# baker-laboratory/NA-MPNN

Hardware: AMD Instinct MI355X
Metric: residues/sec (enc+dec fwd), N~1000 K=48 h=128; seq-recovery vs CPU ref (higher is better)
Workload: dtype f32; 1 GPU; cfg2: B=1 x N=1000 residues per rank, K=48, H=128, 3 enc + 3 dec layers, per-edge GEMMs fp32, seeded random-init weights, independent complexes per rank; precision=fp32, global_batch=1, seq_len=1000, parallelism=replicas x1

## Files before the change

### na_mpnn_amd/csrc/namp.hip

```cpp
#include "../../include/namp.h"
#include "namp_kernels.h"
#include <atomic>
#include "namp_bf16s32.h"
#include "namp_bf16p.h"
#include "namp_node_w.h"
#include "namp_order.h"

#include <cstdarg>
#include <cstdlib>
#include <initializer_list>
#include <cstdio>
#include <mutex>
#include <vector>

namespace {

thread_local char g_err[512] = "";

int fail(int code, const char* fmt, ...) {
  va_list ap;
  va_start(ap, fmt);
  vsnprintf(g_err, sizeof(g_err), fmt, ap);
  va_end(ap);
  return code;
// ... 296 lines not shown
    if (e.npw <= 8 && 2 * e.npw <= e.nwaves) return launch_edge<MODE, 8, PREC_X3, PRE>(a, s);
    return launch_edge<MODE, 16, PREC_X3, PRE>(a, s);
  }
  if (e.npw <= 4) return launch_edge<MODE, 4, PREC_F32, PRE>(a, s);
  if (e.npw <= 8 && 2 * e.npw <= e.nwaves) return launch_edge<MODE, 8, PREC_F32, PRE>(a, s);
  return launch_edge<MODE, 16, PREC_F32, PRE>(a, s);
}

void fill_tail(NodeTail& t, const float* ln1_g, const float* ln1_b, const float* Win_img, const float* b_in,
               const float* Wout_img, const float* b_out, const float* ln2_g, const float* ln2_b, const float* hV,
               const int32_t* mask, float* hV_out, const NampProj* proj, int nproj, const int32_t* S) {
  t.hV = hV; t.mask = mask; t.ln1_g = ln1_g; t.ln1_b = ln1_b; t.Win_img = Win_img; t.b_in = b_in;
  t.Wout_img = Wout_img; t.b_out = b_out; t.ln2_g = ln2_g; t.ln2_b = ln2_b; t.hV_out = hV_out; t.S = S;
  t.head_w = nullptr; t.head_b = nullptr; t.log_probs = nullptr; t.logits = nullptr; t.vocab = 0;
  t.m3_img = nullptr; t.m3_b = nullptr;
  t.nproj = nproj;
  for (int i = 0; i < 8; ++i) {
    if (i < nproj) { t.p[i].img = proj[i].img; t.p[i].bias = proj[i].bias; t.p[i].tok = proj[i].tok; t.p[i].out = proj[i].out; }
    else { t.p[i].img = nullptr; t.p[i].bias = nullptr; t.p[i].tok = nullptr; t.p[i].out = nullptr; }
  }
}

int check_proj(const char* fn, const NampProj* proj, int nproj, const int32_t* S) {
  if (nproj < 0 || nproj > 8 || (nproj > 0 && !proj)) return fail(NAMP_EINVAL, "%s: nproj=%d must be in [0,8]", fn, nproj);
  for (int i = 0; i < nproj; ++i) {
    if (!proj[i].img || !proj[i].out) return fail(NAMP_EINVAL, "%s: proj[%d] has a null image / output", fn, i);
    if (!aligned16(proj[i].img) || !aligned16(proj[i].out) || !aligned16(proj[i].bias) || !aligned16(proj[i].tok))
      return fail(NAMP_EINVAL, "%s: proj[%d] pointers must be 16-byte aligned", fn, i);
    if (proj[i].tok && !S) return fail(NAMP_EINVAL, "%s: proj[%d].tok given but S is null", fn, i);
  }
  return NAMP_OK;
}

struct Out16Req { __bf16* p[8]; int n; bool honoured; };
thread_local Out16Req* g_out16 = nullptr;
thread_local bool g_residue_x1 = false;

int launch_node_linear(const float* X, const int32_t* S, int G_out, int G_src, int N,
                       const NampProj* proj, int nproj, const NampProj* pre, hipStream_t s, bool x3 = false, unsigned* zero = nullptr) {
  NodeLinearArgs a;
  a.X = X; a.S = S; a.G_out = G_out; a.G_src = G_src; a.N = N; a.nproj = nproj; a.zero = zero;
  a.pre.img = pre ? pre->img : nullptr; a.pre.bias = pre ? pre->bias : nullptr;
  a.pre.tok = nullptr; a.pre.out = pre ? pre->out : nullptr;
  for (int i = 0; i < 8; ++i) {
    const NampProj& p = proj[i < nproj ? i : 0];
    a.p[i].img = p.img; a.p[i].bias = p.bias; a.p[i].tok = p.tok; a.p[i].out = p.out;
    a.out16[i] = (g_out16 && i < nproj && i < g_out16->n) ? g_out16->p[i] : nullptr;
    if (a.out16[i]) a.p[i].out = nullptr;
  }
  if (g_out16) g_out16->honoured = true;
  const int units = ((G_out + 15) / 16) * nproj;
  if (x3 && G_out >= 4096 && (g_bf16p.load(std::memory_order_relaxed) & 8) && ensure_attributes() == NAMP_OK) {
    if (g_residue_x1) hipLaunchKernelGGL(node_linear_w_kernel<2>, dim3((G_out + NODEW_ROWS - 1) / NODEW_ROWS), dim3(NODEW_THREADS), NODEW_LDS, s, a);
    else hipLaunchKernelGGL(node_linear_w_kernel<1>, dim3((G_out + NODEW_ROWS - 1) / NODEW_ROWS), dim3(NODEW_THREADS), NODEW_LDS, s, a);
    return NAMP_OK;
  }
  if (x3 && g_residue_x1) hipLaunchKernelGGL(node_linear_kernel<2>, dim3((units + 3) / 4), dim3(256), 0, s, a);
  else if (x3) hipLaunchKernelGGL(node_linear_kernel<1>, dim3((units + 3) / 4), dim3(256), 0, s, a);
  else hipLaunchKernelGGL(node_linear_kernel<0>, dim3((units + 3) / 4), dim3(256), 0, s, a);
  return NAMP_OK;
}

int launch_node_update(const float* ln1_g, const float* ln1_b, const float* Win_img, const float* b_in,
                       const float* Wout_img, const float* b_out, const float* ln2_g, const float* ln2_b,
                       const float* hV, const float* partial, const float* m3_img, const float* m3_b, const int32_t* mask,
                       float* hV_out, const NampProj* proj, int nproj, const int32_t* S, int G, int TPN, hipStream_t s,
// ... 1439 lines not shown
    };
    int cur_ = 0;
    for (int l = 0; l < 3; ++l) {
      const NampEncLayerW* L = &w->enc[l];
      const bool last = (l == 2);
      StageArgs& st = PA_.st[l];
      common(st);
      const int tm = (l & 1) ? 4 : 0, tn = (l & 1) ? 0 : 4, te = (l & 1) ? 6 : 2, tp = (l & 1) ? 2 : 6;
      st.Pa = P[tm]; st.Pj0 = P[tm + 1]; st.Pj1 = nullptr;
      st.W1_img = pick_img(prec, L->W1b_img, nullptr, L->W1b_ximg); st.W2_img = pick_img(prec, L->W2_img, nullptr, L->W2_ximg);
      st.W3_img = pick_img(prec, L->W3_img, nullptr, L->W3_ximg); st.b2 = L->b2; st.b3 = L->b3;
      REQUIRE_PTR(st.W1_img); REQUIRE_PTR(st.W2_img); REQUIRE_PTR(st.W3_img); REQUIRE_PTR(st.b2); REQUIRE_PTR(st.b3);
      if (l == 0) {
        if (E) { st.eW1_img = pick_img(prec, w->We_img, nullptr, w->We_ximg); st.eb2 = w->We_b; REQUIRE_PTR(st.eW1_img); REQUIRE_PTR(st.eb2); }
      } else {
        const NampEncLayerW* Lp = &w->enc[l - 1];
        st.ePa = P[tp]; st.ePj = P[tp + 1];
        st.eW1_img = pick_img(prec, Lp->W11b_img, nullptr, Lp->W11b_ximg); st.eW2_img = pick_img(prec, Lp->W12_img, nullptr, Lp->W12_ximg);
        st.eW3_img = pick_img(prec, Lp->W13_img, nullptr, Lp->W13_ximg); st.eb2 = Lp->b12; st.eb3 = Lp->b13;
        st.ln_g = Lp->ln3_g; st.ln_b = Lp->ln3_b;
        REQUIRE_PTR(st.eW1_img); REQUIRE_PTR(st.eW2_img); REQUIRE_PTR(st.eW3_img); REQUIRE_PTR(st.ln_g); REQUIRE_PTR(st.ln_b);
      }
      st.hE_out = nullptr;
      NampProj pe[8];
      int np = 0;
      pe[np++] = {L->W11a_img, L->b11, nullptr, P[te]};
      pe[np++] = {L->W11c_img, nullptr, nullptr, P[te + 1]};
      if (!last) {
        const NampEncLayerW* Ln = &w->enc[l + 1];
        pe[np++] = {Ln->W1a_img, Ln->b1, nullptr, P[tn]};
        pe[np++] = {Ln->W1c_img, nullptr, nullptr, P[tn + 1]};
      } else {
        const NampDecLayerW* D0 = &w->dec[0];
        for (int d = 0; d < 3; ++d) pe[np++] = {w->dec[d].W1v_img, nullptr, nullptr, Pfw[d]};
        pe[np++] = {D0->W1a_img, D0->b1, nullptr, PA[0]};
        pe[np++] = {D0->W1v_img, nullptr, D0->tok, PB[0]};
      }
      if ((rc = check_proj(__func__, pe, np, S))) return rc;
      fill_tail(st.tail, L->ln1_g, L->ln1_b, L->Win_img, L->b_in, L->Wout_img, L->b_out, L->ln2_g, L->ln2_b, hv[cur_], mask,
                last ? h_V : hv[cur_ ^ 1], pe, np, S);
      st.tail.m3_img = L->W3_img; st.tail.m3_b = L->b3;
      cur_ ^= 1;
    }
    const float* hin_ = h_V;
    for (int l = 0; l < 3; ++l) {
      const NampDecLayerW* D = &w->dec[l];
      StageArgs& st = PA_.st[3 + l];
      common(st);
      st.Pa = PA[l & 1]; st.Pj0 = PB[l & 1]; st.Pj1 = Pfw[l];
      st.W1_img = pick_img(prec, D->W1e_img, nullptr, D->W1e_ximg); st.W2_img = pick_img(prec, D->W2_img, nullptr, D->W2_ximg);
      st.W3_img = pick_img(prec, D->W3_img, nullptr, D->W3_ximg); st.b2 = D->b2; st.b3 = D->b3;
      REQUIRE_PTR(st.W1_img); REQUIRE_PTR(st.W2_img); REQUIRE_PTR(st.W3_img); REQUIRE_PTR(st.b2); REQUIRE_PTR(st.b3);
      if (l == 0) {
        const NampEncLayerW* Lp = &w->enc[2];
        st.ePa = P[2]; st.ePj = P[3];
        st.eW1_img = pick_img(prec, Lp->W11b_img, nullptr, Lp->W11b_ximg); st.eW2_img = pick_img(prec, Lp->W12_img, nullptr, Lp->W12_ximg);
        st.eW3_img = pick_img(prec, Lp->W13_img, nullptr, Lp->W13_ximg); st.eb2 = Lp->b12; st.eb3 = Lp->b13;
        st.ln_g = Lp->ln3_g; st.ln_b = Lp->ln3_b;
        REQUIRE_PTR(st.eW1_img); REQUIRE_PTR(st.eW2_img); REQUIRE_PTR(st.eW3_img); REQUIRE_PTR(st.ln_g); REQUIRE_PTR(st.ln_b);
        st.hE_out = h_E;
      }
      NampProj pn[2] = {{}, {}};
      int np = 0;
      if (l < 2) {
        const NampDecLayerW* Dn = &w->dec[l + 1];
        pn[np++] = {Dn->W1a_img, Dn->b1, nullptr, PA[(l + 1) & 1]};
        pn[np++] = {Dn->W1v_img, nullptr, Dn->tok, PB[(l + 1) & 1]};
      }
      if ((rc = check_proj(__func__, pn, np, S))) return rc;
      fill_tail(st.tail, D->ln1_g, D->ln1_b, D->Win_img, D->b_in, D->Wout_img, D->b_out, D->ln2_g, D->ln2_b, hin_, mask, dhv[l & 1],
                pn, np, S);
      st.tail.m3_img = D->W3_img; st.tail.m3_b = D->b3;
      if (l == 2) { st.tail.head_w = w->Wout_w; st.tail.head_b = w->Wout_b; st.tail.log_probs = log_probs; st.tail.logits = logits; st.tail.vocab = w->vocab; }
      hin_ = dhv[l & 1];
    }
    {
      ProfScope prof_(NAMP_KIND_ENCDEC_PERSISTENT, s);
      if ((rc = namp_internal_launch_persistent(&PA_, prec == PREC_X3 ? 1 : 0, eg.grid, eg.nwaves * 64, s)))
        return fail(NAMP_ELAUNCH, "namp_encdec_fwd: persistent launch setup failed (%d)", rc);
    }
    CHECK_LAUNCH();
    persist_mark(s, pdev);
    return NAMP_OK;
  }
  int cur = 0;
  for (int l = 0; l < w->n_enc; ++l) {
    const NampEncLayerW* L = &w->enc[l];
    const bool last = (l + 1 == w->n_enc);
    float* out = last ? h_V : hv[cur ^ 1];
    const int tm = (l & 1) ? 4 : 0, tn = (l & 1) ? 0 : 4, te = (l & 1) ? 6 : 2, tp = (l & 1) ? 2 : 6;
    NampProj pe[8];
    int np = 0;
    pe[np++] = {L->W11a_img, L->b11, nullptr, P[te]};
    pe[np++] = {L->W11c_img, nullptr, nullptr, P[te + 1]};
    if (!last) {
      const NampEncLayerW* Ln = &w->enc[l + 1];
      pe[np++] = {Ln->W1a_img, Ln->b1, nullptr, P[tn]};
      pe[np++] = {Ln->W1c_img, nullptr, nullptr, P[tn + 1]};
    } else {
      const NampDecLayerW* D0 = &w->dec[0];
      for (int d = 0; d < w->n_dec; ++d) pe[np++] = {w->dec[d].W1v_img, nullptr, nullptr, Pfw[d]};
      pe[np++] = {D0->W1a_img, D0->b1, nullptr, PA[0]};
      pe[np++] = {D0->W1v_img, nullptr, D0->tok, PB[0]};
    }
    if ((rc = check_proj(__func__, pe, np, S))) return rc;
    EdgeArgs a = {};
    a.hE = h_E; a.E_idx = E_idx; a.mask = mask; a.Pa = P[tm]; a.Pj0 = P[tm + 1];
    a.W1_img = pick_img(prec, L->W1b_img, nullptr, L->W1b_ximg); a.W2_img = pick_img(prec, L->W2_img, nullptr, L->W2_ximg);
    a.W3_img = pick_img(prec, L->W3_img, nullptr, L->W3_ximg); a.b2 = L->b2; a.b3 = L->b3;
    REQUIRE_PTR(a.W1_img); REQUIRE_PTR(a.W2_img); REQUIRE_PTR(a.W3_img);
    a.G = a.G_enc = G; a.N = N; a.K = K;
    fill_tail(a.tail, L->ln1_g, L->ln1_b, L->Win_img, L->b_in, L->Wout_img, L->b_out, L->ln2_g, L->ln2_b, hv[cur], mask, out,
              pe, np, S);
    a.tail.m3_img = L->W3_img; a.tail.m3_b = L->b3;
    if (l == 0 && E) {
      a.hE = E; a.hE_out = h_E; a.eW1_img = pick_img(prec, w->We_img, nullptr, w->We_ximg); a.eb2 = w->We_b;
      REQUIRE_PTR(a.eW1_img);
      ProfScope prof_(NAMP_KIND_ENC_MESSAGE, s);
      rc = launch_edge_tail_fused<MODE_ENC_MSG, PRE_EMBED>(a, prec, s);
    } else if (l == 0) {
      ProfScope prof_(NAMP_KIND_ENC_MESSAGE, s);
      rc = launch_edge_tail<MODE_ENC_MSG>(a, prec, s);
    } else {
      const NampEncLayerW* Lp = &w->enc[l - 1];
      a.hE_out = h_E; a.ePa = P[tp]; a.ePj = P[tp + 1];
      a.eW1_img = pick_img(prec, Lp->W11b_img, nullptr, Lp->W11b_ximg); a.eW2_img = pick_img(prec, Lp->W12_img, nullptr, Lp->W12_ximg);
      a.eW3_img = pick_img(prec, Lp->W13_img, nullptr, Lp->W13_ximg); a.eb2 = Lp->b12; a.eb3 = Lp->b13;
      REQUIRE_PTR(a.eW1_img); REQUIRE_PTR(a.eW2_img); REQUIRE_PTR(a.eW3_img);
      a.ln_g = Lp->ln3_g; a.ln_b = Lp->ln3_b;
      ProfScope prof_(NAMP_KIND_ENC_EDGE_MESSAGE, s);
      rc = launch_edge_tail_fused<MODE_ENC_MSG>(a, prec, s);
    }
    if (rc) return rc;
    CHECK_LAUNCH();
    cur ^= 1;
  }
  const int te_last = ((w->n_enc - 1) & 1) ? 6 : 2;
  const float* hin = h_V;
  for (int l = 0; l < w->n_dec; ++l) {
    const NampDecLayerW* D = &w->dec[l];
    const bool last = (l + 1 == w->n_dec);
    float* out = dhv[l & 1];
    NampProj pn[2] = {{}, {}};
    int np = 0;
    if (!last) {
      const NampDecLayerW* Dn = &w->dec[l + 1];
      pn[0] = {Dn->W1a_img, Dn->b1, nullptr, PA[(l + 1) & 1]};
// ... 126 lines not shown
```

### na_mpnn_amd/csrc/namp_kernels.h

```cpp
#pragma once
#include "namp_device.h"
#ifndef NAMP_MAX_LAYERS
#define NAMP_MAX_LAYERS 8
#endif

static __global__ void pack_image_kernel(const float* __restrict__ W, int ld, int col0, int OUT, int IN,
                                  float* __restrict__ img) {
  const int total = OUT * IN;
  for (int e = blockIdx.x * blockDim.x + threadIdx.x; e < total; e += gridDim.x * blockDim.x) {
    const int r = e & 3, lane = (e >> 2) & 63, t = e >> 8;
    const int ntn = OUT >> 4;
    const int tn = t % ntn, tk = t / ntn;
    const int n = 16 * tn + (lane & 15), k = 16 * tk + 4 * (lane >> 4) + r;
    img[e] = W[(size_t)n * ld + col0 + k];
  }
}

static __global__ void pack_image_bf16_kernel(const float* __restrict__ W, int ld, int col0, __bf16* __restrict__ img) {
  const int e = blockIdx.x * blockDim.x + threadIdx.x;
  if (e >= 128 * 128) return;
  const int j = e & 7, lane = (e >> 3) & 63, tn = (e >> 9) & 7, s = e >> 12;
  const int n = 16 * tn + (lane & 15), k = 32 * s + 16 * (j >> 2) + 4 * (lane >> 4) + (j & 3);
  img[e] = (__bf16)W[(size_t)n * ld + col0 + k];
}
// ... 88 lines not shown
          const long b = row / NK;
          const long j = b * N + idx[row];
          v[u] = *(const f4*)(nodes + j * C2 + 4 * (s - s1));
        }
      }
    }
#pragma unroll
    for (int u = 0; u < UNROLL; ++u) {
      if (e0 + u * stride < total) __builtin_nontemporal_store(v[u], (f4*)(out + 4 * (base + e0 + u * stride)));
    }
  }
}

static __global__ void gather_cat_scalar_kernel(const float* __restrict__ nodes, const float* __restrict__ nbrs,
                                         const int32_t* __restrict__ idx, float* __restrict__ out,
                                         long rows, int NK, int N, int C1, int C2) {
  const int ct = C1 + C2;
  const long total = rows * ct;
  for (long e = (long)blockIdx.x * blockDim.x + threadIdx.x; e < total; e += (long)gridDim.x * blockDim.x) {
    const long row = e / ct;
    const int c = (int)(e - row * ct);
    out[e] = (c < C1) ? nbrs[row * C1 + c] : nodes[((row / NK) * N + idx[row]) * C2 + (c - C1)];
  }
}

struct ProjDesc {
  const float* img;
  const float* bias;
  const float* tok;
  float* out;
};

struct NodeTail {
  const float* hV;
  const int32_t* mask;
  const float* ln1_g; const float* ln1_b;
  const float* Win_img;
  const float* b_in;
  const float* Wout_img;
  const float* b_out;
  const float* ln2_g; const float* ln2_b;
  float* hV_out;
  const int32_t* S;
  const float* m3_img;
  const float* m3_b;
  const float* head_w;
  const float* head_b;
  float* log_probs;
  float* logits;
  int vocab;
  int nproj;
  ProjDesc p[8];
};

__device__ __forceinline__ void tail_head_row(const NodeTail& a, const float* ybase, const int sc, const int orow,
                                              const int lane) {
  float z = -INFINITY;
  if (lane < a.vocab) {
    const float* w = a.head_w + (long)lane * NAMP_H;
    float s0 = 0.f, s1 = 0.f, s2 = 0.f, s3 = 0.f;
#pragma unroll 8
    for (int c = 0; c < NAMP_H; c += 4) {
      const f4 wv = *(const f4*)(w + c);
      s0 = fmaf(wv.x, ybase[(c + 0) * sc], s0); s1 = fmaf(wv.y, ybase[(c + 1) * sc], s1);
      s2 = fmaf(wv.z, ybase[(c + 2) * sc], s2); s3 = fmaf(wv.w, ybase[(c + 3) * sc], s3);
    }
    z = (s0 + s1) + (s2 + s3) + a.head_b[lane];
  }
  float mx = z;
#pragma unroll
  for (int o = 1; o < 64; o <<= 1) mx = fmaxf(mx, __shfl_xor(mx, o));
  float e = (lane < a.vocab) ? expf(z - mx) : 0.f;
#pragma unroll
  for (int o = 1; o < 64; o <<= 1) e += __shfl_xor(e, o);
  if (lane < a.vocab) {
    a.log_probs[(long)orow * a.vocab + lane] = (z - mx) - logf(e);
    if (a.logits) a.logits[(long)orow * a.vocab + lane] = z;
  }
}

#define FFN_LD 132
#define NODE_TAIL_LDS ((16 + 16 + 8 * 16) * FFN_LD * 4)
// ... 438 lines not shown
      if (orw >= 0) tail_head_row(a, yT + n, R, orw, lane);
    }
  }
  f4 xr[NB][8];
  tail4_x<NB>(xr, yB, lane);
  int orw[NB];
#pragma unroll
  for (int nb = 0; nb < NB; ++nb) orw[nb] = orow(4 * nb + j);
  auto proj_out = [&](const f4 (&o)[NB], const float* bias, const float* tok, float* out, const int tn) {
    if (!st_lane) return;
    const int c = 16 * tn + 4 * cb;
    const f4 b = bias ? *(const f4*)(bias + c) : (f4){0.f, 0.f, 0.f, 0.f};
#pragma unroll
    for (int nb = 0; nb < NB; ++nb) {
      if (orw[nb] < 0) continue;
      f4 r = o[nb] + b;
      if (tok) r += *(const f4*)(tok + (long)a.S[orw[nb]] * NAMP_H + c);
      float* dst = out + (long)orw[nb] * NAMP_H + c;
      if (SC1) { st_out<true>(dst, r.x); st_out<true>(dst + 1, r.y); st_out<true>(dst + 2, r.z); st_out<true>(dst + 3, r.w); }
      else *(f4*)dst = r;
    }
  };
  if constexpr (PF) {
    tail_units<true>(wave, 8 * (a.nproj < 2 ? a.nproj : 2), nwaves, lane,
                     [&](const int v, const int tk) { return (const f4*)((v >> 3) ? a.p[1].img : a.p[0].img) + (tk * 8 + (v & 7)) * 64; },
                     [&](const int v, const f4 (&wf)[8]) {
                       const bool second = (v >> 3) != 0;
                       f4 o[NB];
                       tail4_unit<NB>(o, wf, xr);
                       proj_out(o, second ? a.p[1].bias : a.p[0].bias, second ? a.p[1].tok : a.p[0].tok, second ? a.p[1].out : a.p[0].out, v & 7);
                     });
    return;
  }
#pragma unroll
  for (int pi = 0; pi < 8; ++pi) {
    if (pi >= a.nproj) break;
    const ProjDesc pd = a.p[pi];
    bool first = AHEAD && pi < TAIL4_AHEAD;
#pragma unroll 1
    for (int tn = ((wave - pi * 8) % nwaves + nwaves) % nwaves; tn < 8; tn += nwaves) {
      f4 o[NB];
      if (first) {
        tail4_unit<NB>(o, wa[pi < TAIL4_AHEAD ? pi : 0], xr);
      } else {
        f4 wf[8];
#pragma unroll
        for (int tk = 0; tk < 8; ++tk) wf[tk] = ((const f4*)pd.img)[(tk * 8 + tn) * 64 + lane];
        tail4_unit<NB>(o, wf, xr);
      }
      first = false;
      proj_out(o, pd.bias, pd.tok, pd.out, tn);
    }
  }
}

template <int R, typename RowFn, bool SC1 = false, bool M3 = true, bool PF = false, bool AH = false>
__device__ __forceinline__ void node_tail_rows(const NodeTail& a, f4 (&x)[8], const float wsum_m, const RowFn orow, float* lds,
                                               const int tid, const int wave, const int nwaves, const int lane) {
#ifndef NAMP_TAIL_VALU
  node_tail_mfma4<R, RowFn, SC1, M3, PF, AH>(a, x, wsum_m, orow, lds, tid, wave, nwaves, lane);
  return;
#endif
  float* xT = lds;
  float* hT = xT + 128 * R;
  float* oP = hT + 512 * R;
  float* yT = oP + 4 * 128 * R;
  float* red = yT + 128 * R;
  const int m = lane & 15, g = lane >> 4;

  if (M3 && a.m3_img) {
    if (wave == 0 && m < R) {
#pragma unroll
      for (int t = 0; t < 8; ++t) {
        xT[(16 * t + 4 * g + 0) * R + m] = x[t].x; xT[(16 * t + 4 * g + 1) * R + m] = x[t].y;
        xT[(16 * t + 4 * g + 2) * R + m] = x[t].z; xT[(16 * t + 4 * g + 3) * R + m] = x[t].w;
      }
      if (g == 0) red[m] = wsum_m;
    }
    __syncthreads();
#pragma unroll 1
    for (int tn = wave; tn < 8; tn += nwaves) {
      f4 wf[8];
#pragma unroll
      for (int tk = 0; tk < 8; ++tk) wf[tk] = ((const f4*)a.m3_img)[(tk * 8 + tn) * 64 + lane];
// ... 264 lines not shown
    }
  }
  if (a.nproj > 0) {
#pragma unroll
    for (int s = 0; s < 4; ++s) split_x3(x[2 * s], x[2 * s + 1], xh[s], xm[s]);
#pragma unroll
    for (int pi = 0; pi < 2; ++pi) {
      if (pi >= a.nproj) break;
      const bf8* wp = (const bf8*)(pi ? p1_p : p0_p) + lane;
      const int tn = wave;
      bf8 f[8];
#pragma unroll
      for (int s = 0; s < 4; ++s) { f[2 * s] = wp[(s * 8 + tn) * 64]; f[2 * s + 1] = wp[NAMP_BIMG_BYTES / 16 + (s * 8 + tn) * 64]; }
      f4 acc = a.p[pi].bias ? *(const f4*)(a.p[pi].bias + 16 * tn + 4 * g) : (f4){0.f, 0.f, 0.f, 0.f};
#pragma unroll
      for (int s = 0; s < 4; ++s) acc = mfma_x3(f[2 * s], f[2 * s + 1], xh[s], xm[s], acc);
      if (orw >= 0) {
        if (a.p[pi].tok) acc += *(const f4*)(a.p[pi].tok + (long)a.S[orw] * NAMP_H + 16 * tn + 4 * g);
        st_f4<SC1>(a.p[pi].out + (long)orw * NAMP_H + 16 * tn + 4 * g, acc);
      }
    }
  }
}

enum { MODE_ENC_MSG = 0, MODE_DEC_MSG = 1, MODE_ENC_EDGE = 2, MODE_EMBED = 3 };

typedef __bf16 bf4 __attribute__((ext_vector_type(4)));
__device__ __forceinline__ int frag_off(const int t, const int g) { return 16 * t + 8 * (g & 1) + 4 * (g >> 1); }
__device__ __forceinline__ void st_frag4(__bf16* row, const int t, const int g, const f4 v) {
  *(bf4*)(row + frag_off(t, g)) = (bf4){(__bf16)v.x, (__bf16)v.y, (__bf16)v.z, (__bf16)v.w};
}

struct EdgeArgs {
  const float* hE;
  float* hE_out;
  const int32_t* E_idx;
  const int32_t* mask;
  const int32_t* mask_attend;
  const int32_t* rank;
  const float* Pa;
  const float* Pj0;
  const float* Pj1;
  const float* W1_img;
  const float* W2_img;
  const float* W3_img;
  const float* b1;
  const float* b2;
  const float* b3;
  const float* ln_g;
  const float* ln_b;
  const float* ePa; const float* ePj;
  const float* eW1_img; const float* eW2_img; const float* eW3_img;
  const float* eb2; const float* eb3;
  uint32_t drop_thresh, drop_seed; float drop_scale;
  const __bf16* hE16; __bf16* hE16_out;
  const __bf16* Pa16; const __bf16* Pj016; const __bf16* Pj116;
  float* partial;
  NodeTail tail;
  int G;
  int G_enc;
  int N, K, TPN;
};

#define EDGE_TAIL_LDS (2 * NAMP_IMG_BYTES + 12 * NAMP_H * 4 + 64 + 2048)

enum { PRE_NONE = 0, PRE_EMBED = 1, PRE_EDGE = 3 };
enum { PREC_F32 = 0, PREC_BF16 = 1, PREC_X3 = 2 };
template <int MODE, int TAIL, int PREC, int PRE, int PERSIST, class Args>
__device__ __forceinline__ void edge_stage(const Args& a, f4 (&x)[8], char* smem) {
  f4 l2pf0 = (f4){0.f, 0.f, 0.f, 0.f}, l2pf1 = l2pf0;
  constexpr bool BF16 = (PREC == PREC_BF16);
  constexpr bool X3 = (PREC == PREC_X3);
  static_assert(PRE == PRE_NONE || (!BF16 && TAIL != 0 && (MODE == MODE_ENC_MSG || MODE == MODE_DEC_MSG)), "PRE: fp32-class message + tail only");
  constexpr bool FUSE = (PRE == PRE_EDGE);
  constexpr bool MSG = (MODE == MODE_ENC_MSG || MODE == MODE_DEC_MSG);
  constexpr bool M3_LDS = MSG && !BF16 && (TAIL == 4 || TAIL == 8);
  char* buf0 = smem;
  char* buf1 = smem + NAMP_IMG_BYTES;
  const int tid = threadIdx.x;
  const int lane = tid & 63;
  const int wave = __builtin_amdgcn_readfirstlane(tid >> 6);
  const int nwaves = blockDim.x >> 6;

  const int m = lane & 15, g = lane >> 4;
  const int npw = nwaves / a.TPN;
  const int node_l = wave / a.TPN, kt = wave - node_l * a.TPN;
  const int bid = xcd_block_index(blockIdx.x, gridDim.x);
  int node = bid * npw + node_l;
  const bool wave_active = (node_l < npw) && (node < a.G);
  if (!wave_active) node = 0;
  const int b_dec = node / a.N;
  const int i_loc = node - b_dec * a.N;
  const int node_enc = (MODE == MODE_DEC_MSG) ? ((b_dec % (a.G_enc / a.N)) * a.N + i_loc) : node;
  const int k = 16 * kt + m;
  const bool valid = wave_active && (k < a.K);
  const long erow = (long)node_enc * a.K + (valid ? k : 0);

  f4 acc[8];
  f4 ybuf[8];
  f4 (&y)[8] = PERSIST ? ybuf : x;
  f4 pjv[8];
  float w_row = 0.f;
  if (PERSIST != 2) {
    const float* src = a.hE + erow * NAMP_H + 4 * g;
#pragma unroll
    for (int t = 0; t < 8; ++t) x[t] = *(const f4*)(src + 16 * t);
  }
  if (MODE == MODE_EMBED) {
    if (a.ln_g) layernorm_row_T(x, a.ln_g, a.ln_b, g);
// ... 33 lines not shown

  const f4* w0 = (const f4*)buf0 + lane;
  const f4* w1 = (const f4*)buf1 + lane;

  if (BF16) {
    const bf8* bw = (const bf8*)smem + lane;
    dma_to_lds(smem, a.W1_img, 32, wave, nwaves, lane);
    if (MODE != MODE_EMBED) dma_to_lds(smem + NAMP_BIMG_BYTES, a.W2_img, 32, wave, nwaves, lane);
    if (MODE == MODE_ENC_EDGE) dma_to_lds(smem + 2 * NAMP_BIMG_BYTES, a.W3_img, 32, wave, nwaves, lane);
    wait_dma_and_sync();
    chain_gemm_bf16<false, false>(acc, x, bw);
    if (MODE != MODE_EMBED) {
#pragma unroll
      for (int t = 0; t < 8; ++t) acc[t] += pjv[t];
      if (MSG) {
#pragma unroll
        for (int t = 0; t < 8; ++t) { const float b = a.b2[16 * t + m]; y[t] = (f4){b, b, b, b}; }
        chain_gemm_bf16<true, true>(y, acc, bw + (NAMP_BIMG_BYTES / 16));
      } else {
#pragma unroll
        for (int t = 0; t < 8; ++t) y[t] = *(const f4*)(a.b2 + 16 * t + 4 * g);
        chain_gemm_bf16<false, true>(y, acc, bw + (NAMP_BIMG_BYTES / 16));
      }
    }
  } else {
  float* cstf = (float*)(smem + 2 * NAMP_IMG_BYTES + 12 * NAMP_H * 4 + 64);
  if (FUSE) {
    dma_to_lds(buf1, a.eW1_img, 64, wave, nwaves, lane);
    dma_to_lds(buf0, a.eW2_img, 64, wave, nwaves, lane);
    for (int i = tid; i < 512; i += (int)blockDim.x) {
      const float* srcv = i < 128 ? a.eb2 : i < 256 ? a.eb3 : i < 384 ? a.ln_g : a.ln_b;
      cstf[i] = srcv[i & 127];
    }
    wait_dma_and_sync();
    gemm128<X3, false, false>(acc, x, w1);
#pragma unroll
    for (int t = 0; t < 8; ++t) acc[t] += pjv[t];
    __syncthreads();
    dma_to_lds(buf1, a.eW3_img, 64, wave, nwaves, lane);
#pragma unroll
    for (int t = 0; t < 8; ++t) pjv[t] = *(const f4*)(cstf + 16 * t + 4 * g);
    gemm128<X3, false, true>(pjv, acc, w0);
    wait_dma_and_sync();
    dma_to_lds(buf0, a.W1_img, 64, wave, nwaves, lane);
#pragma unroll
    for (int t = 0; t < 8; ++t) acc[t] = *(const f4*)(cstf + 128 + 16 * t + 4 * g);
    gemm128<X3, false, true>(acc, pjv, w1);
#pragma unroll
    for (int t = 0; t < 8; ++t) x[t] += acc[t];
    layernorm_row_T(x, cstf + 256, cstf + 384, g);
    if (valid && (PERSIST == 0 || a.hE_out != nullptr)) {
      float* dst = a.hE_out + erow * NAMP_H + 4 * g;
#pragma unroll
      for (int t = 0; t < 8; ++t) *(f4*)(dst + 16 * t) = x[t];
    }
  }
  if (PRE != PRE_NONE) {
    if (PRE == PRE_EMBED) {
      dma_to_lds(buf1, a.eW1_img, 64, wave, nwaves, lane);
      dma_to_lds(buf0, a.W1_img, 64, wave, nwaves, lane);
#pragma unroll
      for (int t = 0; t < 8; ++t) acc[t] = *(const f4*)(a.eb2 + 16 * t + 4 * g);
      wait_dma_and_sync();
      gemm128<X3, false, false>(acc, x, w1);
#pragma unroll
      for (int t = 0; t < 8; ++t) x[t] = acc[t];
      if (valid && (PERSIST == 0 || a.hE_out != nullptr)) {
        float* dst = a.hE_out + erow * NAMP_H + 4 * g;
#pragma unroll
        for (int t = 0; t < 8; ++t) *(f4*)(dst + 16 * t) = x[t];
      }
    }
    {
      const int j_loc = a.E_idx[erow];
      const float* pj;
      if (MODE == MODE_DEC_MSG) {
        const int j_dec = b_dec * a.N + j_loc;
        const bool bw = a.rank[j_dec] < a.rank[node];
        pj = bw ? (a.Pj0 + (long)j_dec * NAMP_H) : (a.Pj1 + (long)(node_enc - i_loc + j_loc) * NAMP_H);
        w_row = valid ? (1.0f / 30.0f) : 0.f;
      } else {
        const int j = node - i_loc + j_loc;
        pj = a.Pj0 + (long)j * NAMP_H;
        int ma;
        if (a.mask_attend) ma = a.mask_attend[erow];
        else ma = a.mask ? (a.mask[node] * a.mask[j]) : 1;
        w_row = valid ? ((float)ma * (1.0f / 30.0f)) : 0.f;
      }
      const float* pa = a.Pa + (long)node * NAMP_H + 4 * g;
      pj += 4 * g;
#pragma unroll
      for (int t = 0; t < 8; ++t) { acc[t] = *(const f4*)(pa + 16 * t); pjv[t] = *(const f4*)(pj + 16 * t); }
    }
    if (PRE == PRE_EMBED) __syncthreads();
    else wait_dma_and_sync();
    dma_to_lds(buf1, a.W2_img, 64, wave, nwaves, lane);
  } else {
  dma_to_lds(buf0, a.W1_img, 64, wave, nwaves, lane);
  if (MODE != MODE_EMBED) dma_to_lds(buf1, a.W2_img, 64, wave, nwaves, lane);
  wait_dma_and_sync();
  }
  gemm128<X3, false, false>(acc, x, w0);

  if (MODE != MODE_EMBED) {
#pragma unroll
  for (int t = 0; t < 8; ++t) acc[t] += pjv[t];
  if (MSG) {
    if (PRE != PRE_NONE) wait_dma_and_sync();
    else if (M3_LDS) __syncthreads();
    if (M3_LDS) dma_to_lds(buf0, a.W3_img, 64, wave, nwaves, lane);
    if (TAIL == 4 || TAIL == 8) {
      const int slice = (blockIdx.x >> 3) & 31;
      const f4* p0; const f4* p1;
      if (wave < 8) {
        p0 = (const f4*)a.tail.Win_img + (slice * 8 + wave) * 64; p1 = (const f4*)a.tail.Wout_img + (slice * 8 + wave) * 64;
      } else {
        const int q = wave - 8;
        const float* img = q == 0 ? a.tail.p[0].img : q == 1 ? a.tail.p[1].img : q == 2 ? a.tail.p[2].img : a.tail.p[3].img;
        if (q >= a.tail.nproj) img = a.tail.Win_img;
        p0 = (const f4*)img + (slice * 2) * 64; p1 = p0 + 64;
      }
      l2pf0 = p0[lane]; l2pf1 = p1[lane];
    }
#pragma unroll
    for (int t = 0; t < 8; ++t) { const float b = a.b2[16 * t + m]; y[t] = (f4){b, b, b, b}; }
    gemm128<X3, true, true>(y, acc, w1);
  } else {
  if (PRE != PRE_NONE) wait_dma_and_sync();
  else __syncthreads();
  dma_to_lds(buf0, a.W3_img, 64, wave, nwaves, lane);

#pragma unroll
// ... 132 lines not shown
  unsigned spins = 0;
  while (__hip_atomic_load(word, __ATOMIC_RELAXED, __HIP_MEMORY_SCOPE_AGENT) < target) {
    __builtin_amdgcn_s_sleep(2);
    if (++spins > NAMP_SPIN_LIMIT) {
      __hip_atomic_store(tmo, code, __ATOMIC_RELAXED, __HIP_MEMORY_SCOPE_AGENT);
      return false;
    }
  }
  return true;
}

__device__ __forceinline__ void grid_barrier(unsigned* sync, const unsigned epoch, const int tid) {
  asm volatile("s_waitcnt vmcnt(0)" ::: "memory");
  __syncthreads();
  if (tid == 0) {
    gu32* sy = (gu32*)sync;
    const int grp = blockIdx.x % NAMP_SYNC_GROUPS;
    const unsigned ngroups = gridDim.x < NAMP_SYNC_GROUPS ? gridDim.x : NAMP_SYNC_GROUPS;
    const unsigned in_group = (gridDim.x - grp + NAMP_SYNC_GROUPS - 1) / NAMP_SYNC_GROUPS;
    const unsigned old = __hip_atomic_fetch_add(sy + grp, 1u, __ATOMIC_RELAXED, __HIP_MEMORY_SCOPE_AGENT);
    if (old + 1 == in_group * epoch) {
      __hip_atomic_fetch_add(sy + NAMP_SYNC_TOP, 1u, __ATOMIC_RELAXED, __HIP_MEMORY_SCOPE_AGENT);
      spin_until_ge(sy + NAMP_SYNC_TOP, ngroups * epoch, sy + NAMP_SYNC_TIMEOUT, 0x10000000u | epoch);
      __hip_atomic_store(sy + NAMP_SYNC_GEN + grp, epoch, __ATOMIC_RELAXED, __HIP_MEMORY_SCOPE_AGENT);
    } else {
      spin_until_ge(sy + NAMP_SYNC_GEN + grp, epoch, sy + NAMP_SYNC_TIMEOUT, 0x20000000u | epoch);
    }
    __builtin_amdgcn_fence(__ATOMIC_ACQUIRE, "agent");
  }
  __syncthreads();
}

struct StageArgs {
  const float* hE; float* hE_out; const int32_t* E_idx; const int32_t* mask; const int32_t* rank;
  const float* Pa; const float* Pj0; const float* Pj1;
  const float* W1_img; const float* W2_img; const float* W3_img; const float* b2; const float* b3;
  const float* ln_g; const float* ln_b;
  const float* ePa; const float* ePj; const float* eW1_img; const float* eW2_img; const float* eW3_img;
  const float* eb2; const float* eb3;
  NodeTail tail;
  int G, G_enc, N, K, TPN;
  static constexpr const int32_t* mask_attend = nullptr;
  static constexpr const float* b1 = nullptr;
  static constexpr uint32_t drop_thresh = 0, drop_seed = 0;
  static constexpr float drop_scale = 1.0f;
  static constexpr const __bf16* hE16 = nullptr;
  static constexpr __bf16* hE16_out = nullptr;
  static constexpr float* partial = nullptr;
};

struct PersistArgs {
  StageArgs st[6];
  unsigned* sync;
  int embed;
};

__device__ __forceinline__ const PersistArgs* persist_kernargs() {
  return (const PersistArgs*)__builtin_amdgcn_kernarg_segment_ptr();
}

template <int TAIL, int PREC>
__global__ __launch_bounds__(768) void encdec_persistent_kernel(const PersistArgs) {
  extern __shared__ __attribute__((aligned(16))) char smem[];
  const PersistArgs* P = persist_kernargs();
  const int tid = threadIdx.x;
  f4 x[8];
  if (P->embed) edge_stage<MODE_ENC_MSG, TAIL, PREC, PRE_EMBED, 1>(P->st[0], x, smem);
  else          edge_stage<MODE_ENC_MSG, TAIL, PREC, PRE_NONE, 1>(P->st[0], x, smem);
  grid_barrier(P->sync, 1, tid);
  edge_stage<MODE_ENC_MSG, TAIL, PREC, PRE_EDGE, 2>(P->st[1], x, smem);
  grid_barrier(P->sync, 2, tid);
  edge_stage<MODE_ENC_MSG, TAIL, PREC, PRE_EDGE, 2>(P->st[2], x, smem);
  grid_barrier(P->sync, 3, tid);
  edge_stage<MODE_DEC_MSG, TAIL, PREC, PRE_EDGE, 2>(P->st[3], x, smem);
// ... 773 lines not shown
  const long off = (long)(valid ? row : 0) * NAMP_H + 4 * g;
  f4 acc[8];
#pragma unroll
  for (int t = 0; t < 8; ++t) acc[t] = (f4){0.f, 0.f, 0.f, 0.f};
#pragma unroll
  for (int q = 0; q < 8; ++q) {
    if (q >= a.n) break;
    f4 x[8];
#pragma unroll
    for (int t = 0; t < 8; ++t) x[t] = *(const f4*)(a.X[q] + off + 16 * t);
    if constexpr (X3) chain_gemm_global_x3<X3 == 2>(acc, x, (const bf8*)a.img[q] + lane);
    else chain_gemm_global<8, 8, false>(acc, x, (const f4*)a.img[q] + lane, 8);
  }
  if (valid) {
    float* dst = a.out + (long)row * NAMP_H + 4 * g;
#pragma unroll
    for (int t = 0; t < 8; ++t) *(f4*)(dst + 16 * t) = acc[t];
  }
}

struct NodeLinearArgs {
  const float* X;
  const int32_t* S;
  int G_out, G_src, N;
  int nproj;
  ProjDesc pre;
  ProjDesc p[8];
  unsigned* zero;
  __bf16* out16[8];
};

template <int X3>
__global__ __launch_bounds__(256) void node_linear_kernel(const NodeLinearArgs a) {
  const int lane = threadIdx.x & 63;
  const int wave = __builtin_amdgcn_readfirstlane(threadIdx.x >> 6);
  const int unit = blockIdx.x * 4 + wave;
  const int ntiles = (a.G_out + 15) >> 4;
  if (a.zero && blockIdx.x == 0 && threadIdx.x < 64) a.zero[threadIdx.x] = 0u;
  if (unit >= ntiles * a.nproj) return;
  const int tile = unit / a.nproj, pi = unit - tile * a.nproj;
  const int m = lane & 15, g = lane >> 4;
  const int row = tile * 16 + m;
  const bool valid = row < a.G_out;
  const int rr = valid ? row : 0;
  const int b = rr / a.N;
  const int src_row = (b % (a.G_src / a.N)) * a.N + (rr - b * a.N);
  ProjDesc d = a.p[0];
  __bf16* o16 = a.out16[0];
#pragma unroll
  for (int q = 1; q < 8; ++q) if (pi == q) { d = a.p[q]; o16 = a.out16[q]; }

  f4 x[8], acc[8];
  const float* src = a.X + (long)src_row * NAMP_H + 4 * g;
#pragma unroll
  for (int t = 0; t < 8; ++t) x[t] = *(const f4*)(src + 16 * t);
  if (a.pre.img) {
#pragma unroll
    for (int t = 0; t < 8; ++t) acc[t] = a.pre.bias ? *(const f4*)(a.pre.bias + 16 * t + 4 * g) : (f4){0.f, 0.f, 0.f, 0.f};
    if constexpr (X3) chain_gemm_global_x3<X3 == 2>(acc, x, (const bf8*)a.pre.img + lane);
    else chain_gemm_global<8, 8, false>(acc, x, (const f4*)a.pre.img + lane, 8);
    if (pi == 0 && valid && a.pre.out) {
      float* dst = a.pre.out + (long)row * NAMP_H + 4 * g;
#pragma unroll
      for (int t = 0; t < 8; ++t) *(f4*)(dst + 16 * t) = acc[t];
    }
#pragma unroll
    for (int t = 0; t < 8; ++t) x[t] = acc[t];
  }
#pragma unroll
  for (int t = 0; t < 8; ++t) acc[t] = d.bias ? *(const f4*)(d.bias + 16 * t + 4 * g) : (f4){0.f, 0.f, 0.f, 0.f};
  if constexpr (X3) chain_gemm_global_x3<X3 == 2>(acc, x, (const bf8*)d.img + lane);
  else chain_gemm_global<8, 8, false>(acc, x, (const f4*)d.img + lane, 8);
  if (d.tok) {
    const float* tk = d.tok + (long)a.S[rr] * NAMP_H + 4 * g;
#pragma unroll
    for (int t = 0; t < 8; ++t) acc[t] += *(const f4*)(tk + 16 * t);
  }
  if (valid && d.out) {
    float* dst = d.out + (long)row * NAMP_H + 4 * g;
#pragma unroll
    for (int t = 0; t < 8; ++t) *(f4*)(dst + 16 * t) = acc[t];
  }
  if (valid && o16) {
    __bf16* dst = o16 + (long)row * NAMP_H;
#pragma unroll
    for (int t = 0; t < 8; ++t) st_frag4(dst, t, g, acc[t]);
  }
}
// ... 1062 lines not shown
```

Before: 2.074 million residues/s.

## Reuse decoder W1v projection for token output and prefetch kernarg lines

The last encoder layer's tail no longer runs a separate W1v GEMM just to add the token embedding for PB[0]. It adds a second-output slot (p[7]) that writes the same Pfw[0] projection result with the token term into PB[0], removing one 128x128 projection per node. The EdgeArgs, StageArgs and NodeTail structs are reordered so fields read early sit together. Non-persistent edge kernels and node_linear touch every kernarg cache line at entry so scalar loads warm the lines before they are needed. This adds inline-asm register holds and a conditional path that depends on rows_tail geometry.

```diff
diff --git a/na_mpnn_amd/csrc/namp.hip b/na_mpnn_amd/csrc/namp.hip
--- a/na_mpnn_amd/csrc/namp.hip
+++ b/na_mpnn_amd/csrc/namp.hip
@@ -352,6 +352,14 @@
   return NAMP_OK;
 }
 
+bool rows_tail(const EdgeGeom& e) { return e.npw <= 4 || (e.npw <= 8 && 2 * e.npw <= e.nwaves); }
+int tail_second_output(const char* fn, NodeTail& t, const float* bias, const float* tok, float* out) {
+  if (t.nproj < 1 || t.nproj > 7 || !out || (tok && !t.S)) return fail(NAMP_EINVAL, "%s: second output needs 1..7 projections, an output and S", fn);
+  if (!aligned16(out) || !aligned16(bias) || !aligned16(tok)) return fail(NAMP_EINVAL, "%s: second-output pointers must be 16-byte aligned", fn);
+  t.p[7].img = nullptr; t.p[7].bias = bias; t.p[7].tok = tok; t.p[7].out = out;
+  return NAMP_OK;
+}
+
 struct Out16Req { __bf16* p[8]; int n; bool honoured; };
 thread_local Out16Req* g_out16 = nullptr;
 thread_local bool g_residue_x1 = false;
@@ -1857,13 +1865,14 @@
         pe[np++] = {Ln->W1c_img, nullptr, nullptr, P[tn + 1]};
       } else {
         const NampDecLayerW* D0 = &w->dec[0];
-        for (int d = 0; d < 3; ++d) pe[np++] = {w->dec[d].W1v_img, nullptr, nullptr, Pfw[d]};
+        for (int d = 1; d < 3; ++d) pe[np++] = {w->dec[d].W1v_img, nullptr, nullptr, Pfw[d]};
         pe[np++] = {D0->W1a_img, D0->b1, nullptr, PA[0]};
-        pe[np++] = {D0->W1v_img, nullptr, D0->tok, PB[0]};
+        pe[np++] = {D0->W1v_img, nullptr, nullptr, Pfw[0]};
       }
       if ((rc = check_proj(__func__, pe, np, S))) return rc;
       fill_tail(st.tail, L->ln1_g, L->ln1_b, L->Win_img, L->b_in, L->Wout_img, L->b_out, L->ln2_g, L->ln2_b, hv[cur_], mask,
                 last ? h_V : hv[cur_ ^ 1], pe, np, S);
+      if (last && (rc = tail_second_output(__func__, st.tail, nullptr, w->dec[0].tok, PB[0]))) return rc;
       st.tail.m3_img = L->W3_img; st.tail.m3_b = L->b3;
       cur_ ^= 1;
     }
@@ -1924,9 +1933,10 @@
       pe[np++] = {Ln->W1c_img, nullptr, nullptr, P[tn + 1]};
     } else {
       const NampDecLayerW* D0 = &w->dec[0];
-      for (int d = 0; d < w->n_dec; ++d) pe[np++] = {w->dec[d].W1v_img, nullptr, nullptr, Pfw[d]};
+      for (int d = 1; d < w->n_dec; ++d) pe[np++] = {w->dec[d].W1v_img, nullptr, nullptr, Pfw[d]};
       pe[np++] = {D0->W1a_img, D0->b1, nullptr, PA[0]};
-      pe[np++] = {D0->W1v_img, nullptr, D0->tok, PB[0]};
+      pe[np++] = {D0->W1v_img, nullptr, nullptr, Pfw[0]};
+      if (!rows_tail(eg)) pe[np++] = {D0->W1v_img, nullptr, D0->tok, PB[0]};
     }
     if ((rc = check_proj(__func__, pe, np, S))) return rc;
     EdgeArgs a = {};
@@ -1938,6 +1948,7 @@
     fill_tail(a.tail, L->ln1_g, L->ln1_b, L->Win_img, L->b_in, L->Wout_img, L->b_out, L->ln2_g, L->ln2_b, hv[cur], mask, out,
               pe, np, S);
     a.tail.m3_img = L->W3_img; a.tail.m3_b = L->b3;
+    if (last && rows_tail(eg) && (rc = tail_second_output(__func__, a.tail, nullptr, w->dec[0].tok, PB[0]))) return rc;
     if (l == 0 && E) {
       a.hE = E; a.hE_out = h_E; a.eW1_img = pick_img(prec, w->We_img, nullptr, w->We_ximg); a.eb2 = w->We_b;
       REQUIRE_PTR(a.eW1_img);
diff --git a/na_mpnn_amd/csrc/namp_kernels.h b/na_mpnn_amd/csrc/namp_kernels.h
--- a/na_mpnn_amd/csrc/namp_kernels.h
+++ b/na_mpnn_amd/csrc/namp_kernels.h
@@ -144,22 +144,22 @@
 };
 
 struct NodeTail {
+  const float* m3_img;
+  const float* m3_b;
   const float* hV;
-  const int32_t* mask;
   const float* ln1_g; const float* ln1_b;
   const float* Win_img;
   const float* b_in;
   const float* Wout_img;
   const float* b_out;
   const float* ln2_g; const float* ln2_b;
+  const int32_t* mask;
   float* hV_out;
-  const int32_t* S;
-  const float* m3_img;
-  const float* m3_b;
   const float* head_w;
   const float* head_b;
   float* log_probs;
   float* logits;
+  const int32_t* S;
   int vocab;
   int nproj;
   ProjDesc p[8];
@@ -664,6 +664,8 @@
                      });
     return;
   }
+  const ProjDesc p2 = a.p[7];
+  const bool two = !p2.img && p2.out;
 #pragma unroll
   for (int pi = 0; pi < 8; ++pi) {
     if (pi >= a.nproj) break;
@@ -682,6 +684,7 @@
       }
       first = false;
       proj_out(o, pd.bias, pd.tok, pd.out, tn);
+      if (two && pi + 1 == a.nproj) proj_out(o, p2.bias, p2.tok, p2.out, tn);
     }
   }
 }
@@ -1012,35 +1015,53 @@
 }
 
 struct EdgeArgs {
+  int G;
+  int G_enc;
+  int N, K, TPN;
   const float* hE;
+  const int32_t* E_idx;
+  const float* ePa; const float* ePj;
   float* hE_out;
-  const int32_t* E_idx;
-  const int32_t* mask;
-  const int32_t* mask_attend;
-  const int32_t* rank;
+  const float* eW1_img; const float* eW2_img; const float* eW3_img;
+  const float* eb2; const float* eb3;
+  const float* ln_g;
+  const float* ln_b;
+  const float* W1_img;
   const float* Pa;
   const float* Pj0;
   const float* Pj1;
-  const float* W1_img;
+  const int32_t* rank;
+  const int32_t* mask;
+  const int32_t* mask_attend;
   const float* W2_img;
   const float* W3_img;
+  const float* b2;
+  NodeTail tail;
   const float* b1;
-  const float* b2;
   const float* b3;
-  const float* ln_g;
-  const float* ln_b;
-  const float* ePa; const float* ePj;
-  const float* eW1_img; const float* eW2_img; const float* eW3_img;
-  const float* eb2; const float* eb3;
   uint32_t drop_thresh, drop_seed; float drop_scale;
   const __bf16* hE16; __bf16* hE16_out;
   const __bf16* Pa16; const __bf16* Pj016; const __bf16* Pj116;
   float* partial;
-  NodeTail tail;
-  int G;
-  int G_enc;
-  int N, K, TPN;
 };
+
+template <class Args>
+struct KernargLines {
+  static constexpr int N = ((int)sizeof(Args) + 63) / 64 + 1;
+  uint32_t v[N];
+};
+template <class Args>
+__device__ __forceinline__ void kernarg_touch(KernargLines<Args>& k) {
+  const uint32_t* seg = (const uint32_t*)__builtin_amdgcn_kernarg_segment_ptr();
+#pragma unroll
+  for (int i = 0; i + 1 < KernargLines<Args>::N; ++i) k.v[i] = seg[16 * i];
+  k.v[KernargLines<Args>::N - 1] = seg[sizeof(Args) / 4 - 1];
+}
+template <class Args>
+__device__ __forceinline__ void kernarg_retire(const KernargLines<Args>& k) {
+#pragma unroll
+  for (int i = 0; i < KernargLines<Args>::N; ++i) asm volatile("" :: "s"(k.v[i]));
+}
 
 #define EDGE_TAIL_LDS (2 * NAMP_IMG_BYTES + 12 * NAMP_H * 4 + 64 + 2048)
 
@@ -1055,6 +1076,9 @@
   constexpr bool FUSE = (PRE == PRE_EDGE);
   constexpr bool MSG = (MODE == MODE_ENC_MSG || MODE == MODE_DEC_MSG);
   constexpr bool M3_LDS = MSG && !BF16 && (TAIL == 4 || TAIL == 8);
+  constexpr bool WARM = (PERSIST == 0) && !BF16 && (TAIL == 4 || TAIL == 8);
+  KernargLines<Args> kargs;
+  if constexpr (WARM) kernarg_touch(kargs);
   char* buf0 = smem;
   char* buf1 = smem + NAMP_IMG_BYTES;
   const int tid = threadIdx.x;
@@ -1154,6 +1178,7 @@
       const float* srcv = i < 128 ? a.eb2 : i < 256 ? a.eb3 : i < 384 ? a.ln_g : a.ln_b;
       cstf[i] = srcv[i & 127];
     }
+    if constexpr (WARM) kernarg_retire(kargs);
     wait_dma_and_sync();
     gemm128<X3, false, false>(acc, x, w1);
 #pragma unroll
@@ -1183,6 +1208,7 @@
       dma_to_lds(buf0, a.W1_img, 64, wave, nwaves, lane);
 #pragma unroll
       for (int t = 0; t < 8; ++t) acc[t] = *(const f4*)(a.eb2 + 16 * t + 4 * g);
+      if constexpr (WARM) kernarg_retire(kargs);
       wait_dma_and_sync();
       gemm128<X3, false, false>(acc, x, w1);
 #pragma unroll
@@ -1220,6 +1246,7 @@
   } else {
   dma_to_lds(buf0, a.W1_img, 64, wave, nwaves, lane);
   if (MODE != MODE_EMBED) dma_to_lds(buf1, a.W2_img, 64, wave, nwaves, lane);
+  if constexpr (WARM) kernarg_retire(kargs);
   wait_dma_and_sync();
   }
   gemm128<X3, false, false>(acc, x, w0);
@@ -1418,14 +1445,13 @@
 }
 
 struct StageArgs {
-  const float* hE; float* hE_out; const int32_t* E_idx; const int32_t* mask; const int32_t* rank;
-  const float* Pa; const float* Pj0; const float* Pj1;
-  const float* W1_img; const float* W2_img; const float* W3_img; const float* b2; const float* b3;
-  const float* ln_g; const float* ln_b;
-  const float* ePa; const float* ePj; const float* eW1_img; const float* eW2_img; const float* eW3_img;
-  const float* eb2; const float* eb3;
+  int G, G_enc, N, K, TPN;
+  const float* hE; const int32_t* E_idx; const float* ePa; const float* ePj; float* hE_out;
+  const float* eW1_img; const float* eW2_img; const float* eW3_img; const float* eb2; const float* eb3;
+  const float* ln_g; const float* ln_b; const float* W1_img;
+  const float* Pa; const float* Pj0; const float* Pj1; const int32_t* rank; const int32_t* mask;
+  const float* W2_img; const float* W3_img; const float* b2; const float* b3;
   NodeTail tail;
-  int G, G_enc, N, K, TPN;
   static constexpr const int32_t* mask_attend = nullptr;
   static constexpr const float* b1 = nullptr;
   static constexpr uint32_t drop_thresh = 0, drop_seed = 0;
@@ -2265,6 +2291,8 @@
 
 template <int X3>
 __global__ __launch_bounds__(256) void node_linear_kernel(const NodeLinearArgs a) {
+  KernargLines<NodeLinearArgs> kargs;
+  kernarg_touch(kargs);
   const int lane = threadIdx.x & 63;
   const int wave = __builtin_amdgcn_readfirstlane(threadIdx.x >> 6);
   const int unit = blockIdx.x * 4 + wave;
@@ -2287,6 +2315,7 @@
   const float* src = a.X + (long)src_row * NAMP_H + 4 * g;
 #pragma unroll
   for (int t = 0; t < 8; ++t) x[t] = *(const f4*)(src + 16 * t);
+  kernarg_retire(kargs);
   if (a.pre.img) {
 #pragma unroll
     for (int t = 0; t < 8; ++t) acc[t] = a.pre.bias ? *(const f4*)(a.pre.bias + 16 * t + 4 * g) : (f4){0.f, 0.f, 0.f, 0.f};
```

New measurement: 2.081 million residues/s, median of 6. No clear change (+0.3%).
